# worldfnd/provekit

Measured on AMD Instinct MI355X. Metric: proofs/sec (noir-r1cs prove hot path, WHIR commit + sumcheck + folding rounds), higher is better.
Workload: dtype u32x8 (BN254-Fr, 256-bit Montgomery integers); 1 GPU; poseidon-rounds size class: m=21, m_0=20, satisfiable synthetic R1CS (786429 constraints, 1048571 witnesses, a constant term in half of the rows of A and B), batch-2 WHIR commit + zk-sumcheck + 4-round WHIR opening, queries [109, 28, 16, 11]/9, pow_bits [19.0, 16.0, 16.0, 18.0]/11.0 (WhirConfig::new derivation, security 128, ConjectureList), blinding WHIR n=8 queries [122]/31, Skyscraper-sponge tr; launcher=single process

## Files before the change

### provekit_amd/csrc/internal.hpp

```cpp
#pragma once
#include "ctx.hpp"
#include "rng_core.hpp"

namespace pk {

int ensure_scratch(pk_ctx* ctx, size_t bytes);
int ensure_pinned(pk_ctx* ctx);
int ensure_ws(pk_ctx* ctx, size_t bytes);
enum { PK_HOOK_GATE_SPINS = 0, PK_HOOK_GATE_STALL_US = 1, PK_HOOK_RCCL_SAME_DEVICE = 2, PK_HOOK_COUNT = 3 };
long test_hook(int which);
hipError_t wait_stream(int device, hipStream_t stream);
hipError_t wait_ctx(pk_ctx* ctx);
int wait_ctx_rc(pk_ctx* ctx);
int sync_stream(pk_ctx* ctx);
int mail_alloc(pk_ctx* ctx, size_t bytes, void** out);

int comm_rank(const pk_ctx* ctx);
int comm_world(const pk_ctx* ctx);
int comm_all_gather(pk_ctx* ctx, const void* d_send, void* d_recv, size_t bytes_per_rank);
int comm_all_reduce_sum_u64(pk_ctx* ctx, uint64_t* d_buf, size_t count);
int comm_collect_fe(pk_ctx* ctx, int K, uint64_t* host_out);
int red_across_begin(pk_ctx* ctx);
bool comm_collective_pending(const pk_ctx* ctx);
bool comm_rccl(const pk_ctx* ctx);
hipError_t comm_wait(pk_ctx* ctx);
void comm_turn_begin(pk_ctx* ctx);
void comm_turn_end(pk_ctx* ctx);
unsigned long long comm_collectives_issued(const pk_ctx* ctx);
void comm_abort(pk_ctx* ctx);
void comm_release(pk_ctx* ctx);

int leaf_hash_x(pk_ctx* ctx, const uint64_t* d_leaves, size_t n_leaves, size_t width, uint64_t* d_digests, bool scaled_in);
int merkle_top_x(pk_ctx* ctx, uint64_t* d_nodes, size_t top_leaves);
int read_root(pk_ctx* ctx, const uint64_t* d_nodes, size_t n_leaves, uint64_t root[4]);

void ntt_retain_ctx(pk_ctx* ctx);
void ntt_release_ctx(pk_ctx* ctx);
bool ntt_scaled_available(unsigned log_n);
int rs_encode_x(pk_ctx* ctx, const uint64_t* const* d_coeffs, unsigned batch, unsigned n_vars, unsigned log_inv_rate, unsigned fold,
                uint64_t* d_leaves, uint64_t* d_scratch, bool scaled);
int rs_encode_shard_x(pk_ctx* ctx, const uint64_t* const* d_coeffs, unsigned batch, unsigned n_vars, unsigned log_inv_rate, unsigned fold,
                      unsigned shard, unsigned n_shards, uint64_t* d_leaves_local, uint64_t* d_scratch, bool scaled);

int pow_solve_x(pk_ctx* ctx, const uint8_t challenge[32], double bits, uint64_t* nonce, bool striped);

unsigned shard_factor(const pk_ctx* ctx, size_t rows);
size_t commit_scratch_fes(const pk_ctx* ctx, size_t rows, size_t width);
int commit_into(pk_ctx* ctx, const uint64_t* const* d_coeffs, unsigned batch, unsigned n_vars, unsigned log_inv_rate, unsigned fold,
                uint64_t* d_leaves, uint64_t* d_nodes, uint64_t* d_scratch, pk_commit_layout* layout_out);
int open_raw(pk_ctx* ctx, const uint64_t* d_leaves, const uint64_t* d_nodes, size_t n_leaves, size_t width, const pk_commit_layout& lay,
             const uint64_t* indices, size_t k, int canonical_leaves, uint64_t* leaves_out, uint64_t* sibling_digests, uint64_t* auth_paths);

int eval_univariate_multi(pk_ctx* ctx, const uint64_t* const* d_polys, unsigned np, size_t n, const uint64_t z[4], uint64_t* out);
int dot_rows(pk_ctx* ctx, const uint64_t* d_w, size_t row_stride, unsigned nrows, const uint64_t* d_f, const uint64_t* d_g, size_t n, uint64_t* out,
             bool defer = false);
int lincomb2(pk_ctx* ctx, uint64_t* d_out, const uint64_t* d_a, const uint64_t* beta, const uint64_t* d_b, size_t n);
int lincomb2_pair(pk_ctx* ctx, uint64_t* d_out0, const uint64_t* d_a0, const uint64_t* d_b0, size_t n0, uint64_t* d_out1, const uint64_t* d_a1,
                  const uint64_t* d_b1, size_t n1, const uint64_t* beta);
int axpy3(pk_ctx* ctx, uint64_t* d_y, const uint64_t* g3, const uint64_t* d_rows, size_t row_stride, size_t n);
int to_coeffs_generated(pk_ctx* ctx, unsigned m, const uint64_t* d_wit, size_t n_wit, const RngKey& key, uint32_t stream_mask, uint32_t stream_g,
                        uint64_t* d_f_evals, uint64_t* d_g_evals, uint64_t* d_f_coeffs, uint64_t* d_g_coeffs);
int fold_pairs2(pk_ctx* ctx, const uint64_t* d_v0, uint64_t* d_out0, const uint64_t* d_v1, uint64_t* d_out1, size_t len, const uint64_t* r,
                unsigned gate_seq = 0);
enum class CubicWeight { EqArray, Level };
int sumcheck_cubic_launch(pk_ctx* ctx, uint64_t* d_a, uint64_t* d_b, uint64_t* d_c, CubicWeight kind, uint64_t* d_weight, size_t len,
                          const uint64_t* fold_or_null, unsigned gate_seq, unsigned* red_seq_out);
int sumcheck_quadratic_launch(pk_ctx* ctx, const uint64_t* d_f, const uint64_t* d_w, size_t len, const uint64_t* fold_or_null, unsigned gate_seq,
                              uint64_t* d_f_out, uint64_t* d_w_out, int nsums, unsigned* red_seq_out);
void sumcheck_quadratic_from_claim(const uint64_t claim[4], uint64_t out[12]);
int eq_suffix_tables(pk_ctx* ctx, const uint64_t* r, unsigned n, uint64_t* d_out);
void sumcheck_spliteq_correct(const uint64_t P[4], const uint64_t r_i[4], uint64_t out[12]);
void sumcheck_spliteq_advance(uint64_t P[4], const uint64_t r_i[4], const uint64_t alpha_i[4]);
int sumcheck_collect_spin(pk_ctx* ctx, int nsums, unsigned red_seq, uint64_t out[12]);
int sumcheck_collect(pk_ctx* ctx, int nsums, uint64_t out[12]);
unsigned sumcheck_gate_next(pk_ctx* ctx);
void sumcheck_gate_publish(pk_ctx* ctx, unsigned gate_seq, const uint64_t challenge[4]);
int sumcheck_gate_check(pk_ctx* ctx);
void sumcheck_gate_clear(pk_ctx* ctx);

int witness_bounds_strided(pk_ctx* ctx, const pk_r1cs* r, const uint64_t* d_z, unsigned m0, unsigned stride, unsigned offset, uint64_t* d_a,
                           uint64_t* d_b, uint64_t* d_c);
int external_row_range(pk_ctx* ctx, const pk_r1cs* r, const uint64_t* d_eq_alpha, size_t first, size_t last, uint64_t* d_out);

enum { RNG_MASK = 1, RNG_G = 2, RNG_BLIND = 3, RNG_MASK_B = 4, RNG_G_B = 5, RNG_FILL = 6 };
int proof_key(pk_ctx* ctx, const uint8_t* rng_seed32, RngKey& key);
int random_fe(pk_ctx* ctx, uint64_t* d_out, size_t n, const RngKey& key, uint32_t stream);

void witness_program_shape(const pk_witness_program* p, size_t* n_witnesses, size_t* n_challenges, size_t* n_acir);
// ... 13 lines not shown
```

### provekit_amd/csrc/mle.hip

```cpp
#define PK_BASE_PRIO 2
#include "internal.hpp"
#include "fe29.hpp"
#include "reduce.hpp"

using namespace pk;

namespace {

struct fe_arg {
    u32 v[8];
};
__device__ __forceinline__ fe from_arg(const fe_arg& a) {
    fe r;
#pragma unroll
    for (int i = 0; i < 8; i++) r.v[i] = a.v[i];
    return r;
}
inline fe_arg to_arg(const uint64_t* h) {
    fe_arg a;
    memcpy(a.v, h, 32);
    return a;
}

__device__ __forceinline__ fe lds_get(const uint4* lo, const uint4* hi, int i) {
// ... 310 lines not shown
    PK_LATENCY_PRIO();
    static_assert(NS == 2 || NS == 3, "two or three sums");
    const fe r = (FOLD && gate.host) ? gate_wait(gate) : from_arg(fold_arg);
    fe acc[NS];
#pragma unroll
    for (int q = 0; q < NS; q++) acc[q] = fe_zero();
    const size_t npairs = out_len / 2;
    const size_t stride = (size_t)gridDim.x * blockDim.x;
    for (size_t i = (size_t)blockIdx.x * blockDim.x + threadIdx.x; i < npairs; i += stride) {
        fe f0, f1, w0, w1;
        if (FOLD) {
            fe x0 = fe_load(f + 4 * i), x1 = fe_load(f + 4 * i + 1), x2 = fe_load(f + 4 * i + 2), x3 = fe_load(f + 4 * i + 3);
            f0 = fe_fold(x0, x1, r);
            f1 = fe_fold(x2, x3, r);
            fe y0 = fe_load(w + 4 * i), y1 = fe_load(w + 4 * i + 1), y2 = fe_load(w + 4 * i + 2), y3 = fe_load(w + 4 * i + 3);
            w0 = fe_fold(y0, y1, r);
            w1 = fe_fold(y2, y3, r);
            fe_store(f_out + 2 * i, f0);
            fe_store(f_out + 2 * i + 1, f1);
            fe_store(w_out + 2 * i, w0);
            fe_store(w_out + 2 * i + 1, w1);
        } else {
            f0 = fe_load(f + 2 * i);
            f1 = fe_load(f + 2 * i + 1);
            w0 = fe_load(w + 2 * i);
            w1 = fe_load(w + 2 * i + 1);
        }
        acc[0] = fe_add(acc[0], fe_mulx(f0, w0));
        if (NS == 3) acc[1] = fe_add(acc[1], fe_mulx(f1, w1));
        acc[NS - 1] = fe_add(acc[NS - 1], fe_mulx(fe_sub(fe_dbl(f1), f0), fe_sub(fe_dbl(w1), w0)));
    }
    grid_finish_fe<NS>(acc, red);
}
constexpr size_t SMALL_ROUND_PAIRS = 16384;
constexpr unsigned EQ_SUFFIX_ONE_WG_VARS = 11;

template <CubicWeight W>
__device__ __forceinline__ void cubic_round_small(fe* __restrict__ a, fe* __restrict__ b, fe* __restrict__ c, weight_elem<W>* __restrict__ wt, size_t len,
                                                  fe_arg fold_arg, gate_args gate, red_out red) {
    constexpr bool LEVEL = W == CubicWeight::Level;
    PK_LATENCY_PRIO();
    __shared__ uint4 xs[2 * RED_THREADS];
    const fe alpha = gate.host ? gate_wait(gate) : from_arg(fold_arg);
    const size_t npairs = len / 4, off = npairs, foff = len / 2;
    const unsigned tid = threadIdx.x, g = tid >> 3, role = tid & 7, k = role >> 1, which = role & 1;
    const size_t i = (size_t)blockIdx.x * (RED_THREADS / 8) + g;
    fe* arr = k == 0 ? a : k == 1 ? b : c;
    if constexpr (!LEVEL) arr = k == 0 ? a : k == 1 ? b : k == 2 ? c : wt;
    if (i < npairs && (!LEVEL || k < 3)) {
        fe* p = arr + i + (which ? off : 0);
        fe x = fe_load(p), x2 = fe_load(p + foff);
        x = fe_fold(x, x2, alpha);
        fe_store(p, x);
        lds_put(xs, xs + RED_THREADS, tid, x);
    } else if (LEVEL && i < npairs && role == 6) {
        lds_put(xs, xs + RED_THREADS, tid, fe_load(wt + i));
    }
    __syncthreads();
    fe acc[3] = {fe_zero(), fe_zero(), fe_zero()};
    if (i < npairs && role < 3) {
        const unsigned base = tid & ~7u;
        auto v = [&](unsigned kk, unsigned w) { return lds_get(xs, xs + RED_THREADS, base + 2 * kk + w); };
        const fe a0 = v(0, 0), a1 = v(0, 1), b0 = v(1, 0), b1 = v(1, 1), c0 = v(2, 0), c1 = v(2, 1), e0 = v(3, 0);
        fe e1;
        if constexpr (!LEVEL) e1 = v(3, 1);
        auto pick = [&](const fe& x0, const fe& x1) {
// ... 116 lines not shown
                                                                                   red_out red) {
    cubic_round_small<CubicWeight::Level>(a, b, c, E, len, fold_arg, gate, red);
}

__global__ void fold_pairs_kernel(const fe* __restrict__ v0, fe* __restrict__ out0, const fe* __restrict__ v1, fe* __restrict__ out1,
                                  size_t out_len, fe_arg r_arg, gate_args gate) {
    PK_LATENCY_PRIO();
    const fe r = gate.host ? gate_wait(gate) : from_arg(r_arg);
    const fe* v = blockIdx.y ? v1 : v0;
    fe* out = blockIdx.y ? out1 : out0;
    const size_t stride = (size_t)gridDim.x * blockDim.x;
    for (size_t i = (size_t)blockIdx.x * blockDim.x + threadIdx.x; i < out_len; i += stride) {
        fe x0 = fe_load(v + 2 * i), x1 = fe_load(v + 2 * i + 1);
        fe_store(out + i, fe_fold(x0, x1, r));
    }
}

template <int NV>
__global__ __launch_bounds__(RED_THREADS) void dot_kernel(const fe* __restrict__ w, const fe* __restrict__ f, const fe* __restrict__ g,
                                                          size_t n, red_out red) {
    PK_LATENCY_PRIO();
    fe acc[NV];
#pragma unroll
    for (int k = 0; k < NV; k++) acc[k] = fe_zero();
    const size_t stride = (size_t)gridDim.x * blockDim.x;
    for (size_t i = (size_t)blockIdx.x * blockDim.x + threadIdx.x; i < n; i += stride) {
        fe wi = fe_load(w + i);
        acc[0] = fe_add(acc[0], fe_mulx(wi, fe_load(f + i)));
        if (NV == 2) acc[NV - 1] = fe_add(acc[NV - 1], fe_mulx(wi, fe_load(g + i)));
    }
    grid_finish_fe<NV>(acc, red);
}

template <int NR, int NV>
__global__ __launch_bounds__(RED_THREADS) void dot_rows_kernel(const fe* __restrict__ w, size_t row_stride, const fe* __restrict__ f,
                                                               const fe* __restrict__ g, size_t n, red_out red) {
    PK_LATENCY_PRIO();
    fe acc[NR * NV];
#pragma unroll
    for (int k = 0; k < NR * NV; k++) acc[k] = fe_zero();
    const size_t stride = (size_t)gridDim.x * blockDim.x;
    for (size_t i = (size_t)blockIdx.x * blockDim.x + threadIdx.x; i < n; i += stride) {
        const fe fi = fe_load(f + i);
        fe gi = fi;
        if (NV == 2) gi = fe_load(g + i);
#pragma unroll
        for (int k = 0; k < NR; k++) {
            const fe wi = fe_load(w + (size_t)k * row_stride + i);
            acc[NV * k] = fe_add(acc[NV * k], fe_mulx(wi, fi));
            if (NV == 2) acc[NV * k + 1] = fe_add(acc[NV * k + 1], fe_mulx(wi, gi));
        }
    }
    grid_finish_fe<NR * NV>(acc, red);
}

struct pow2_args {
    fe_arg p[28];
};
__global__ __launch_bounds__(RED_THREADS) void zpow_table_kernel(pow2_args zp, fe* __restrict__ ztab) {
    PK_LATENCY_PRIO();
    fe h = fe_one();
#pragma unroll 1
    for (int i = 0; i < 8; i++)
        if ((threadIdx.x >> i) & 1u) h = fe_mulx(h, from_arg(zp.p[i]));
    fe_store(ztab + threadIdx.x, h);
}
template <int NP>
__global__ __launch_bounds__(RED_THREADS) void horner_kernel(const fe* __restrict__ c, const fe* __restrict__ c_second, size_t n, size_t cnt, pow2_args zp,
                                                             const fe* __restrict__ ztab, red_out red) {
    PK_LATENCY_PRIO();
    __shared__ unsigned s_zb[8];
    static_assert(RED_THREADS == 256, "the lane table has 256 entries");
    const size_t base = (size_t)blockIdx.x * cnt * RED_THREADS;
    if (threadIdx.x == 0) {
        fe zb = fe_one();
        bool any = false;
// ... 88 lines not shown
        if (j == 0 && t < n_out) fe_store(out + t, wide_reduce(w));
    }
}

__global__ __launch_bounds__(256) void lincomb_kernel(fe* __restrict__ out, const fe* __restrict__ a, const fe* __restrict__ b, size_t n,
                                                      fe_arg beta_arg) {
    PK_LATENCY_PRIO();
    const fe beta = from_arg(beta_arg);
    const size_t stride = (size_t)gridDim.x * blockDim.x;
    for (size_t i = (size_t)blockIdx.x * blockDim.x + threadIdx.x; i < n; i += stride)
        fe_store(out + i, fe_add(fe_load(a + i), fe_mulx(beta, fe_load(b + i))));
}
__global__ __launch_bounds__(256) void axpy_kernel(fe* __restrict__ y, const fe* __restrict__ x, size_t n, fe_arg beta_arg) {
    PK_LATENCY_PRIO();
    const fe beta = from_arg(beta_arg);
    const size_t stride = (size_t)gridDim.x * blockDim.x;
    for (size_t i = (size_t)blockIdx.x * blockDim.x + threadIdx.x; i < n; i += stride)
        fe_store(y + i, fe_add(fe_load(y + i), fe_mulx(beta, fe_load(x + i))));
}

__global__ __launch_bounds__(256) void lincomb_pair_kernel(fe* __restrict__ out0, const fe* __restrict__ a0, const fe* __restrict__ b0, size_t n0,
                                                           fe* __restrict__ out1, const fe* __restrict__ a1, const fe* __restrict__ b1, size_t n1,
                                                           fe_arg beta_arg) {
    PK_LATENCY_PRIO();
    const fe beta = from_arg(beta_arg);
    fe* out = blockIdx.y ? out1 : out0;
    const fe* a = blockIdx.y ? a1 : a0;
    const fe* b = blockIdx.y ? b1 : b0;
    const size_t n = blockIdx.y ? n1 : n0;
    const size_t stride = (size_t)gridDim.x * blockDim.x;
    for (size_t i = (size_t)blockIdx.x * blockDim.x + threadIdx.x; i < n; i += stride)
        fe_store(out + i, fe_add(fe_load(a + i), fe_mulx(beta, fe_load(b + i))));
}
struct fe3_arg {
    fe_arg g[3];
};
__global__ __launch_bounds__(256) void axpy3_kernel(fe* __restrict__ y, const fe* __restrict__ rows, size_t row_stride, size_t n, fe3_arg ga) {
    PK_LATENCY_PRIO();
    const fe29 g0 = unpack29<5>(from_arg(ga.g[0])), g1 = unpack29<5>(from_arg(ga.g[1])), g2 = unpack29<5>(from_arg(ga.g[2]));
    const size_t stride = (size_t)gridDim.x * blockDim.x;
    for (size_t i = (size_t)blockIdx.x * blockDim.x + threadIdx.x; i < n; i += stride) {
        dot29 d;
        dot29_init(d);
        dot29_add(d, unpack29<0>(fe_load(rows + i)), g0);
        dot29_add(d, unpack29<0>(fe_load(rows + row_stride + i)), g1);
        dot29_add(d, unpack29<0>(fe_load(rows + 2 * row_stride + i)), g2);
        fe_store(y + i, fe_add(fe_load(y + i), dot29_result(d)));
    }
}

int dot(pk_ctx* ctx, int nv, const uint64_t* d_w, const uint64_t* d_f, const uint64_t* d_g, size_t n, uint64_t* out) {
    if (n == 0) return reduce_empty(ctx, nv, out);
    red_out red;
    unsigned blocks;
    int rc = reduction_begin(ctx, n, &red, &blocks);
    if (rc) return rc;
    {
        ProfScope prof(ctx, "dot");
        auto kernel = nv == 2 ? dot_kernel<2> : dot_kernel<1>;
        kernel<<<blocks, RED_THREADS, 0, ctx->stream>>>((const fe*)d_w, (const fe*)d_f, (const fe*)d_g, n, red);
    }
    PK_LAUNCH_CHECK(ctx);
    return collect_reduction(ctx, nv, out);
}

struct round_launch {
    red_out red;
    unsigned blocks;
    gate_args gate;
// ... 197 lines not shown
    if (!ctx->d_ztab) PK_HIP(ctx, hipMalloc(&ctx->d_ztab, 256 * 32));
    pow2_args zp;
    {
        fe b;
        memcpy(b.v, z, 32);
        for (int i = 0; i < 28; i++) {
            memcpy(zp.p[i].v, b.v, 32);
            b = fe_mulx(b, b);
        }
    }
    {
        ProfScope prof(ctx, "eval_univariate");
        zpow_table_kernel<<<1, RED_THREADS, 0, ctx->stream>>>(zp, (fe*)ctx->d_ztab);
        auto kernel = np == 2 ? horner_kernel<2> : horner_kernel<1>;
        kernel<<<blocks, RED_THREADS, 0, ctx->stream>>>((const fe*)d_polys[0], (const fe*)(np == 2 ? d_polys[1] : nullptr), n, cnt, zp,
                                                        (const fe*)ctx->d_ztab, red);
    }
    PK_LAUNCH_CHECK(ctx);
    return collect_reduction(ctx, (int)np, out);
}
int dot_rows(pk_ctx* ctx, const uint64_t* d_w, size_t row_stride, unsigned nrows, const uint64_t* d_f, const uint64_t* d_g, size_t n, uint64_t* out,
             bool defer) {
    const int nv = d_g ? 2 : 1;
    PK_REQUIRE(ctx, nrows == 3 && (out || defer) && (n == 0 || (d_w && d_f)), "three weight rows");
    PK_REQUIRE(ctx, !defer || (n != 0 && !ctx->red_across), "a deferred dot product needs work and a lone context");
    if (n == 0) return reduce_empty(ctx, 3 * nv, out);
    red_out red;
    unsigned blocks;
    int rc = reduction_begin(ctx, n, &red, &blocks);
    if (rc) return rc;
    {
        ProfScope prof(ctx, "dot");
        auto kernel = nv == 2 ? dot_rows_kernel<3, 2> : dot_rows_kernel<3, 1>;
        kernel<<<blocks, RED_THREADS, 0, ctx->stream>>>((const fe*)d_w, row_stride, (const fe*)d_f, (const fe*)d_g, n, red);
    }
    PK_LAUNCH_CHECK(ctx);
    if (defer) return PK_OK;
    return collect_reduction(ctx, 3 * nv, out);
}

}

extern "C" {

int pk_to_coeffs(pk_ctx* ctx, uint64_t* d_evals, unsigned n_vars) {
    PK_ENTER(ctx);
    return wavelet<true>(ctx, nullptr, d_evals, n_vars);
}
int pk_to_evals(pk_ctx* ctx, uint64_t* d_coeffs, unsigned n_vars) {
    PK_ENTER(ctx);
    return wavelet<false>(ctx, nullptr, d_coeffs, n_vars);
}
int pk_to_coeffs_into(pk_ctx* ctx, const uint64_t* d_src, uint64_t* d_dst, unsigned n_vars) {
    PK_ENTER(ctx);
    PK_REQUIRE(ctx, d_src && d_src != d_dst, "source must differ from destination");
    return wavelet<true>(ctx, d_src, d_dst, n_vars);
}
int pk_to_evals_into(pk_ctx* ctx, const uint64_t* d_src, uint64_t* d_dst, unsigned n_vars) {
    PK_ENTER(ctx);
    PK_REQUIRE(ctx, d_src && d_src != d_dst, "source must differ from destination");
    return wavelet<false>(ctx, d_src, d_dst, n_vars);
}

int pk_eq_accumulate(pk_ctx* ctx, uint64_t* d_w, unsigned n_vars, const uint64_t* points, const uint64_t* scales, unsigned q,
                     int overwrite) {
    PK_ENTER(ctx);
    PK_REQUIRE(ctx, d_w && (q == 0 || (points && scales)), "null pointer");
    PK_REQUIRE(ctx, n_vars <= 30, "too many variables");
    const size_t n = (size_t)1 << n_vars;
    if (q == 0) {
        if (overwrite) PK_HIP(ctx, hipMemsetAsync(d_w, 0, 32 * n, ctx->stream));
        return PK_OK;
    }
    const unsigned nlo = (n_vars + 1) / 2, nhi = n_vars - nlo;
    const size_t per_pt = ((size_t)1 << nhi) + ((size_t)1 << nlo);
    int rc = ensure_ws(ctx, 32 * (size_t)q * per_pt + 64);
    if (rc) return rc;
    PK_REQUIRE(ctx, nlo <= 16, "too many variables");
    char* mail = nullptr;
    rc = mail_alloc(ctx, 32 * ((size_t)q * n_vars + q), (void**)&mail);
    if (rc) return rc;
    fe* d_points = (fe*)mail;
    fe* d_scales = d_points + (size_t)q * n_vars;
    fe* d_tables = (fe*)ctx->d_ws;
    if (n_vars) memcpy(d_points, points, 32 * (size_t)q * n_vars);
    memcpy(d_scales, scales, 32 * (size_t)q);
    {
        ProfScope prof(ctx, "eq_accumulate");
        eq_half_tables_kernel<<<dim3(q, 2), 256, 0, ctx->stream>>>(d_points, d_scales, n_vars, nhi, nlo, d_tables);
        eq_accumulate_kernel<<<grid_for(ctx, nlo ? (n + 1) / 2 : n, 256), 256, 0, ctx->stream>>>((fe*)d_w, n, nhi, nlo, q, d_tables, overwrite);
    }
    PK_LAUNCH_CHECK(ctx);
    return PK_OK;
}

int pk_eq_table(pk_ctx* ctx, const uint64_t* r, unsigned m, uint64_t* d_out) {
    PK_ENTER(ctx);
    static const uint64_t one[4] = {0xac96341c4ffffffbULL, 0x36fc76959f60cd29ULL, 0x666ea36f7879462eULL, 0x0e0a77c19a07df2fULL};
    return pk_eq_accumulate(ctx, d_out, m, r, one, 1, 1);
}


int pk_sumcheck_cubic_round(pk_ctx* ctx, uint64_t* d_a, uint64_t* d_b, uint64_t* d_c, uint64_t* d_eq, size_t len,
                            const uint64_t* fold_or_null, uint64_t out[12]) {
    PK_ENTER(ctx);
    PK_REQUIRE(ctx, out, "null pointer");
    unsigned seq = 0;
    int rc = sumcheck_cubic_launch(ctx, d_a, d_b, d_c, CubicWeight::EqArray, d_eq, len, fold_or_null, 0, &seq);
    if (rc) return rc;
    return collect_reduction(ctx, 3, out);
}

int pk_sumcheck_quadratic_round(pk_ctx* ctx, const uint64_t* d_f, const uint64_t* d_w, size_t len, const uint64_t* fold_or_null,
                                uint64_t* d_f_out, uint64_t* d_w_out, uint64_t out[12]) {
    PK_ENTER(ctx);
    PK_REQUIRE(ctx, out, "null pointer");
    unsigned seq = 0;
    int rc = sumcheck_quadratic_launch(ctx, d_f, d_w, len, fold_or_null, 0, d_f_out, d_w_out, 3, &seq);
    if (rc) return rc;
    return collect_reduction(ctx, 3, out);
}

// ... 105 lines not shown
```

### provekit_amd/csrc/prover.hip

```cpp
#include <unistd.h>

#include <algorithm>
#include <chrono>
#include <cstdlib>
#include <string>
#include <vector>

#include "internal.hpp"
#include "shard_map.hpp"
#include "prover_transcript.hpp"

using namespace pk;

struct pk_scheme {
    const pk_r1cs* r1cs = nullptr;
    size_t num_constraints = 0, num_witnesses = 0;
    unsigned m = 0, m_0 = 0;
    unsigned nb = 0;
    pk_whir_config whir_witness{}, whir_hiding{};
    char* arena = nullptr;
    size_t arena_bytes = 0;
    std::string domain_separator;
    char* noir_witness = nullptr;
    pk_ctx* side = nullptr;
// ... 280 lines not shown
    const unsigned n, k, G, lgG, rank;
    bool sharded;
    const size_t B0, off0;
    fe* d_c = nullptr;
    fe* bp[2] = {};
    fe* bw[2] = {};
    fe* gathered[4] = {};
    int cur = 0;
    size_t len;
    std::vector<fe> rs;
    fe claim;
    bool have_claim = false;
    std::vector<fe> all_r;

    WhirProver(pk_ctx* c, Arena& a, const pk_whir_config& cf, const Commitment& com, Transcript& t)
        : ctx(c), A(a), cfg(cf), C(com), T(t), n(cf.n_vars), k(cf.folding_factor), G((unsigned)comm_world(c)), lgG(ilog2(G)),
          rank((unsigned)comm_rank(c)), sharded(whir_sharded(c, n)), B0(sharded ? ((size_t)1 << n) / G : (size_t)1 << n),
          off0(sharded ? (size_t)rank * B0 : 0), len(B0) {}

    int batch_combine(fe* dst, fe* const* x, size_t from, size_t cnt) {
        if (C.batch == 1) return pk_memcpy_d2d(ctx, dst, x[0] + from, 32 * cnt);
        uint64_t s[4];
        h_store(s, C.beta);
        int rc = lincomb2(ctx, U(dst), U(x[0] + from), s, U(x[1] + from), cnt);
        fe bp_ = h_mul(C.beta, C.beta);
        for (unsigned b = 2; b < C.batch && !rc; b++) {
            h_store(s, bp_);
            rc = pk_fe_axpy(ctx, U(dst), s, U(x[b] + from), cnt);
            bp_ = h_mul(bp_, C.beta);
        }
        return rc;
    }

    int eq_weights(fe* dst, unsigned nv, const std::vector<fe>& zs, const fe& gamma, int overwrite, fe* next) {
        const size_t q = zs.size();
        const unsigned lg = sharded ? lgG : 0, nl = nv - lg;
        std::vector<fe> x(nv ? nv : 1), pts(q * (nl ? nl : 1)), scales(q ? q : 1);
        fe g = fe_one();
        for (size_t j = 0; j < q; j++) {
            expand_from_univariate(zs[j], nv, x.data());
            scales[j] = lg ? h_mul(g, eq_bits(x.data(), lg, rank)) : g;
            std::copy(x.begin() + lg, x.begin() + nv, pts.begin() + j * nl);
            g = h_mul(g, gamma);
        }
        *next = g;
        return pk_eq_accumulate(ctx, U(dst), nl, (const uint64_t*)pts.data(), (const uint64_t*)scales.data(), (unsigned)q, overwrite);
    }

    void flip() {
        cur = 1 - cur;
        len /= 2;
    }

    int sumcheck_rounds(unsigned rounds) {
        rs.clear();
        ns0 = have_claim ? 2 : 3;
        const bool pipelined = ctx->latency_mode && G == 1 && rounds && len >= ((size_t)1 << rounds);
        return sumcheck_round_loop(ctx, T, rounds, pipelined, *this);
    }
    int ns0 = 3;
    int nsums(unsigned t) const { return t ? 2 : ns0; }
    int launch(unsigned t, const uint64_t* fold, unsigned gate_seq, unsigned* red_seq) {
        CK(sumcheck_quadratic_launch(ctx, U(bp[cur]), U(bw[cur]), len, fold, gate_seq, U(bp[1 - cur]), U(bw[1 - cur]), nsums(t), red_seq));
        if (fold || gate_seq) flip();
        return PK_OK;
    }
    bool closing_fold() const { return len >= 2; }
    int fold(const uint64_t* r, unsigned gate_seq) {
        CK(fold_pairs2(ctx, U(bp[cur]), U(bp[1 - cur]), U(bw[cur]), U(bw[1 - cur]), len, r, gate_seq));
        flip();
        return PK_OK;
    }
    int before_sync_launch() { return PK_OK; }
    void meanwhile(unsigned) {}
    unsigned message(unsigned t, uint64_t out[12], fe msg[4]) {
        if (nsums(t) == 2) {
            uint64_t cl[4];
            h_store(cl, claim);
            sumcheck_quadratic_from_claim(cl, out);
        }
        for (int q = 0; q < 3; q++) msg[q] = h_load(out + 4 * q);
        return 3;
    }
    void record(unsigned, const fe* msg, const fe& r) {
        rs.push_back(r);
        all_r.push_back(r);
        claim = eval_quadratic_012(msg, r);
        have_claim = true;
    }

    int gather(fe* p0, fe* p1, fe* w0, fe* w1) {
        CK(gather_blocks(ctx, bp[cur], len, p0));
        CK(gather_blocks(ctx, bw[cur], len, w0));
        bp[0] = p0; bp[1] = p1; bw[0] = w0; bw[1] = w1;
        cur = 0;
        len *= G;
        sharded = false;
        return PK_OK;
    }
    int maybe_gather() { return sharded && len <= SHARD_MIN_LOCAL ? gather(gathered[0], gathered[1], gathered[2], gathered[3]) : PK_OK; }

    int start(fe* const* d_weights, const size_t* weight_len, unsigned n_weights, const fe* weight_sums) {
        const size_t N = (size_t)1 << n;
        ALLOC(dc, N);
        d_c = dc;
        ALLOC(p0, B0);
        ALLOC(p1, B0 / 2 ? B0 / 2 : 1);
        ALLOC(w0, B0);
        ALLOC(w1, B0 / 2 ? B0 / 2 : 1);
        bp[0] = p0; bp[1] = p1; bw[0] = w0; bw[1] = w1;
        bool have_evals = true;
        for (unsigned b = 0; b < C.batch; b++) have_evals = have_evals && C.evals[b] != nullptr;
        const bool pair = have_evals && C.batch == 2;
        if (pair) {
            uint64_t s[4];
            h_store(s, C.beta);
            CK(lincomb2_pair(ctx, U(d_c), U(C.polys[0]), U(C.polys[1]), N, U(p0), U(C.evals[0] + off0), U(C.evals[1] + off0), B0, s));
        } else {
            CK(batch_combine(d_c, C.polys, 0, N));
        }
        if (have_evals) {
            if (!pair) CK(batch_combine(p0, C.evals, off0, B0));
        } else if (!sharded) {
            CK(pk_to_evals_into(ctx, U(d_c), U(p0), n));
        } else {
            ALLOC(d_ev, N);
            CK(pk_to_evals_into(ctx, U(d_c), U(d_ev), n));
            CK(pk_memcpy_d2d(ctx, p0, d_ev + off0, 32 * B0));
        }
        const fe gamma = T.challenge_scalar();
        fe g;
        CK(eq_weights(w0, n, C.ood_points, gamma, 1, &g));
        auto batched = [&](const fe* v, size_t step) {
            fe acc = v[0], bb = C.beta;
            for (unsigned b = 1; b < C.batch; b++, bb = h_mul(bb, C.beta)) acc = h_add(acc, h_mul(bb, v[b * step]));
            return acc;
        };
        const size_t q = C.ood_points.size();
        claim = fe_zero();
        fe gq = fe_one();
        for (size_t j = 0; j < q; j++, gq = h_mul(gq, gamma)) claim = h_add(claim, h_mul(gq, batched(&C.ood_answers[j], q)));
        have_claim = weight_sums || !n_weights;
        const bool rows3 = rows_at_equal_stride3(d_weights, weight_len, n_weights);
        if (rows3) {
            uint64_t s3[12];
            fe g3 = g;
            for (int i = 0; i < 3; i++, g3 = h_mul(g3, gamma)) h_store(s3 + 4 * i, g3);
            CK(axpy3(ctx, U(w0), s3, U(d_weights[0] + off0), (size_t)(d_weights[1] - d_weights[0]), in_block(weight_len[0], off0, B0)));
        }
        for (unsigned i = 0; i < n_weights; i++) {
            uint64_t s[4];
            h_store(s, g);
            const size_t cnt = in_block(weight_len[i], off0, B0);
            if (cnt && !rows3) CK(pk_fe_axpy(ctx, U(w0), s, U(d_weights[i] + off0), cnt));
            if (weight_sums) claim = h_add(claim, h_mul(g, batched(weight_sums + (size_t)i * C.batch, 1)));
            g = h_mul(g, gamma);
        }
        if (sharded) {
            const size_t cap = G * SHARD_MIN_LOCAL;
            const size_t sizes[4] = {cap, cap / 2, cap, cap / 2};
            for (int q = 0; q < 4; q++) {
                ALLOC(buf, sizes[q]);
                gathered[q] = buf;
            }
        }
        CK(sumcheck_rounds(k));
        return maybe_gather();
    }

    int rounds() {
        const Commitment* prev = &C;
        Commitment com;
        unsigned nv = n, log_inv_rate = cfg.starting_log_inv_rate;
        size_t domain_size = (size_t)1 << (n + log_inv_rate);
        fe exp_gen = folded_domain_generator(n + log_inv_rate, k);
        for (unsigned r = 0; r < cfg.n_rounds; r++) {
            const unsigned nv2 = nv - k;
            ALLOC(d_c2, (size_t)1 << nv2);
            CK(pk_fold_coeffs(ctx, U(d_c), nv, (const uint64_t*)rs.data(), k, U(d_c2)));
            d_c = d_c2;
            nv = nv2;
            log_inv_rate += k - 1;
            Commitment next;
            CK(whir_commit_compute(ctx, A, nv, log_inv_rate, k, &d_c, 1, next));
            fe root;
            CK(read_root(ctx, U(next.nodes), next.rows, (uint64_t*)root.v));
            T.add_canon(root);
            std::vector<fe> zs(cfg.ood_samples[r]);
            T.challenge_scalars(zs.data(), zs.size());
            std::vector<fe> ood_ans(zs.size());
            for (size_t j = 0; j < zs.size(); j++) CK(eval_univariate_x(ctx, d_c, (size_t)1 << nv, zs[j], ood_ans[j]));
            T.add_scalars(ood_ans.data(), ood_ans.size());
            CK(pow_round(ctx, T, cfg.pow_bits[r]));
            const std::vector<uint64_t> idx = stir_queries(T, domain_size, k, cfg.num_queries[r]);
            CK(emit_opening_hints(ctx, T, *prev, idx));
            const fe gamma = T.challenge_scalar();
            for (uint64_t i : idx) zs.push_back(h_pow(exp_gen, i));
            fe g;
            CK(eq_weights(bw[cur], nv, zs, gamma, 0, &g));
            have_claim = false;
            CK(sumcheck_rounds(k));
            CK(maybe_gather());
            com = next;
            prev = &com;
            domain_size /= 2;
            exp_gen = h_mul(exp_gen, exp_gen);
        }
        return final_round(*prev, nv, domain_size);
    }

    int final_round(const Commitment& prev, unsigned nv, size_t domain_size) {
        if (sharded) {
            const size_t cap = len * G;
            ALLOC(fp0, cap);
            ALLOC(fp1, cap / 2 ? cap / 2 : 1);
            ALLOC(fw0, cap);
            ALLOC(fw1, cap / 2 ? cap / 2 : 1);
            CK(gather(fp0, fp1, fw0, fw1));
        }
        const unsigned nv2 = nv - k;
        ALLOC(d_final, (size_t)1 << nv2);
        CK(pk_fold_coeffs(ctx, U(d_c), nv, (const uint64_t*)rs.data(), k, U(d_final)));
        std::vector<fe> fin((size_t)1 << nv2);
        CK(pk_memcpy_d2h(ctx, fin.data(), d_final, 32 * fin.size()));
        T.add_scalars(fin.data(), fin.size());
        CK(pow_round(ctx, T, cfg.final_pow_bits));
        const std::vector<uint64_t> idx = stir_queries(T, domain_size, k, cfg.final_queries);
        CK(emit_opening_hints(ctx, T, prev, idx));
        CK(sumcheck_rounds(nv2));
        return pow_round(ctx, T, cfg.final_folding_pow_bits);
    }

    int deferred_hint(fe* const* d_weights, const size_t* weight_len, unsigned n_weights) {
        if (!n_weights) return PK_OK;
        std::vector<fe> point(all_r.rbegin(), all_r.rend());
        const bool sh = whir_sharded(ctx, n);
        ALLOC(d_eq, B0);
        if (sh) {
            const fe sc = eq_bits(point.data(), lgG, rank);
            CK(pk_eq_accumulate(ctx, U(d_eq), n - lgG, (const uint64_t*)(point.data() + lgG), (const uint64_t*)&sc, 1, 1));
        } else {
            CK(pk_eq_table(ctx, (const uint64_t*)point.data(), n, U(d_eq)));
        }
        Across ac(ctx, sh);
        CK(ac.rc);
        std::vector<fe> evals(n_weights);
        const bool rows3 = rows_at_equal_stride3(d_weights, weight_len, n_weights);
        if (rows3) {
            uint64_t o[12] = {};
            if (sh || weight_len[0])
                CK(dot_rows(ctx, U(d_weights[0] + off0), (size_t)(d_weights[1] - d_weights[0]), 3, U(d_eq), nullptr, in_block(weight_len[0], off0, B0), o));
            for (int i = 0; i < 3; i++) evals[i] = h_load(o + 4 * i);
        } else {
            for (unsigned i = 0; i < n_weights; i++) {
                uint64_t o[4] = {};
                if (sh || weight_len[i]) CK(pk_dot(ctx, U(d_weights[i] + off0), U(d_eq), in_block(weight_len[i], off0, B0), o));
                evals[i] = h_load(o);
            }
        }
        std::vector<uint8_t> buf;
        put_vec(buf, evals.data(), n_weights);
        T.hint(buf.data(), buf.size());
        return PK_OK;
    }
};
int whir_prove(pk_ctx* ctx, Arena& A, const pk_whir_config& cfg, const Commitment& C, fe* const* d_weights, const size_t* weight_len,
               unsigned n_weights, const fe* weight_sums, Transcript& T) {
    WhirProver P(ctx, A, cfg, C, T);
    CK(P.start(d_weights, weight_len, n_weights, weight_sums));
    CK(P.rounds());
    return P.deferred_hint(d_weights, weight_len, n_weights);
}

struct BatchCommit {
    Commitment com;
    fe* f_evals = nullptr;
    fe* g_evals = nullptr;
};
int batch_commit_compute(pk_ctx* ctx, Arena& A, unsigned m, const pk_whir_config& cfg, const fe* d_evals, size_t n_evals, const RngKey& key,
                         u32 stream_mask, u32 stream_g, BatchCommit& out) {
    const size_t half = (size_t)1 << (m - 1), N = 2 * half;
    ALLOC(f, N);
    ALLOC(g, N);
    ALLOC(fe_, N);
    ALLOC(ge_, N);
    if (comm_world(ctx) <= 1) {
        CK(to_coeffs_generated(ctx, m, U(d_evals), n_evals, key, stream_mask, stream_g, U(f), U(g), U(fe_), U(ge_)));
    } else {
        CK(pk_memset_zero(ctx, f, 32 * half));
        CK(pk_memcpy_d2d(ctx, f, d_evals, 32 * n_evals));
// ... 489 lines not shown
```

Before: 286.1 proofs/s.

## Fuse WHIR opening weight build, batch combine and first sumcheck round into one kernel

```diff
diff --git a/provekit_amd/csrc/internal.hpp b/provekit_amd/csrc/internal.hpp
--- a/provekit_amd/csrc/internal.hpp
+++ b/provekit_amd/csrc/internal.hpp
@@ -54,6 +54,22 @@
 int eval_univariate_multi(pk_ctx* ctx, const uint64_t* const* d_polys, unsigned np, size_t n, const uint64_t z[4], uint64_t* out);
 int dot_rows(pk_ctx* ctx, const uint64_t* d_w, size_t row_stride, unsigned nrows, const uint64_t* d_f, const uint64_t* d_g, size_t n, uint64_t* out,
              bool defer = false);
+int dot_rows_eq(pk_ctx* ctx, const uint64_t* d_w, size_t row_stride, unsigned nrows, const uint64_t* point, unsigned n_vars, size_t n, uint64_t* out);
+struct opening_first {
+    const uint64_t *d_e0, *d_e1, *beta;
+    uint64_t *d_p, *d_w;
+    size_t n;
+    const uint64_t *points, *scales;
+    unsigned q;
+    int overwrite;
+    const uint64_t* d_rows;
+    size_t row_stride;
+    unsigned nrows;
+    size_t row_len;
+    const uint64_t* row_scales;
+    int nsums;
+};
+int opening_first_launch(pk_ctx* ctx, const opening_first& a, unsigned grid, unsigned* red_seq_out);
 int lincomb2(pk_ctx* ctx, uint64_t* d_out, const uint64_t* d_a, const uint64_t* beta, const uint64_t* d_b, size_t n);
 int lincomb2_pair(pk_ctx* ctx, uint64_t* d_out0, const uint64_t* d_a0, const uint64_t* d_b0, size_t n0, uint64_t* d_out1, const uint64_t* d_a1,
                   const uint64_t* d_b1, size_t n1, const uint64_t* beta);
diff --git a/provekit_amd/csrc/mle.hip b/provekit_amd/csrc/mle.hip
--- a/provekit_amd/csrc/mle.hip
+++ b/provekit_amd/csrc/mle.hip
@@ -366,6 +366,80 @@
     }
     grid_finish_fe<NS>(acc, red);
 }
+struct fe3_arg {
+    fe_arg g[3];
+};
+struct first_rows {
+    const fe* rows;
+    size_t stride, len;
+    fe3_arg g;
+};
+template <int NR>
+__device__ __forceinline__ fe first_rows_term(const first_rows& R, size_t i) {
+    static_assert(NR == 1 || NR == 3, "one row or three");
+    if constexpr (NR == 1) {
+        return fe_mulx(from_arg(R.g.g[0]), fe_load(R.rows + i));
+    } else {
+        dot29 d;
+        dot29_init(d);
+#pragma unroll
+        for (int k = 0; k < 3; k++) dot29_add(d, unpack29<0>(fe_load(R.rows + k * R.stride + i)), unpack29<5>(from_arg(R.g.g[k])));
+        return dot29_result(d);
+    }
+}
+template <bool COMBINE, int NR, int NS>
+__global__ __launch_bounds__(RED_THREADS) void opening_first_kernel(const fe* __restrict__ e0, const fe* __restrict__ e1, fe_arg beta_arg,
+                                                                    fe* __restrict__ p, fe* __restrict__ w, size_t n, unsigned nhi, unsigned nlo,
+                                                                    unsigned q, const fe* __restrict__ tables, int overwrite, first_rows R, red_out red) {
+    PK_LATENCY_PRIO();
+    static_assert(NS == 2 || NS == 3, "two or three sums");
+    const size_t per_pt = ((size_t)1 << nhi) + ((size_t)1 << nlo);
+    const size_t mask = ((size_t)1 << nlo) - 1;
+    fe acc[NS];
+#pragma unroll
+    for (int s = 0; s < NS; s++) acc[s] = fe_zero();
+    const size_t stride = (size_t)gridDim.x * blockDim.x;
+    for (size_t j = (size_t)blockIdx.x * blockDim.x + threadIdx.x; j < n / 2; j += stride) {
+        const size_t i = 2 * j;
+        dot29 d0, d1;
+        dot29_init(d0);
+        dot29_init(d1);
+        const fe* T = tables;
+        for (unsigned pt = 0; pt < q; pt++, T += per_pt) {
+            const fe29 h = unpack29<0>(fe_load(T + (i >> nlo)));
+            const fe* lo = T + ((size_t)1 << nhi) + (i & mask);
+            dot29_add(d0, h, unpack29<5>(fe_load(lo)));
+            dot29_add(d1, h, unpack29<5>(fe_load(lo + 1)));
+        }
+        fe w0 = dot29_result(d0), w1 = dot29_result(d1);
+        if (!overwrite) {
+            w0 = fe_add(fe_load(w + i), w0);
+            w1 = fe_add(fe_load(w + i + 1), w1);
+        }
+        if constexpr (NR > 0) {
+            if (i < R.len) w0 = fe_add(w0, first_rows_term<NR>(R, i));
+            if (i + 1 < R.len) w1 = fe_add(w1, first_rows_term<NR>(R, i + 1));
+        }
+        fe_store(w + i, w0);
+        fe_store(w + i + 1, w1);
+        fe f0, f1;
+        if constexpr (COMBINE) {
+            const fe beta = from_arg(beta_arg);
+            f0 = fe_add(fe_load(e0 + i), fe_mulx(beta, fe_load(e1 + i)));
+            f1 = fe_add(fe_load(e0 + i + 1), fe_mulx(beta, fe_load(e1 + i + 1)));
+            fe_store(p + i, f0);
+            fe_store(p + i + 1, f1);
+        } else {
+            f0 = fe_load(p + i);
+            f1 = fe_load(p + i + 1);
+        }
+        acc[0] = fe_add(acc[0], fe_mulx(f0, w0));
+        if (NS == 3) acc[1] = fe_add(acc[1], fe_mulx(f1, w1));
+        acc[NS - 1] = fe_add(acc[NS - 1], fe_mulx(fe_sub(fe_dbl(f1), f0), fe_sub(fe_dbl(w1), w0)));
+    }
+    grid_finish_fe<NS>(acc, red);
+}
+
 constexpr size_t SMALL_ROUND_PAIRS = 16384;
 constexpr unsigned EQ_SUFFIX_ONE_WG_VARS = 11;
 
@@ -548,16 +622,19 @@
     grid_finish_fe<NV>(acc, red);
 }
 
-template <int NR, int NV>
+template <int NR, int NV, bool EQF = false>
 __global__ __launch_bounds__(RED_THREADS) void dot_rows_kernel(const fe* __restrict__ w, size_t row_stride, const fe* __restrict__ f,
-                                                               const fe* __restrict__ g, size_t n, red_out red) {
-    PK_LATENCY_PRIO();
+                                                               const fe* __restrict__ g, size_t n, unsigned nhi, unsigned nlo, red_out red) {
+    PK_LATENCY_PRIO();
+    static_assert(!EQF || NV == 1, "the equality table stands in for f alone");
     fe acc[NR * NV];
 #pragma unroll
     for (int k = 0; k < NR * NV; k++) acc[k] = fe_zero();
     const size_t stride = (size_t)gridDim.x * blockDim.x;
     for (size_t i = (size_t)blockIdx.x * blockDim.x + threadIdx.x; i < n; i += stride) {
-        const fe fi = fe_load(f + i);
+        fe fi;
+        if constexpr (EQF) fi = fe_mulx(fe_load(f + (i >> nlo)), fe_load(f + ((size_t)1 << nhi) + (i & (((size_t)1 << nlo) - 1))));
+        else fi = fe_load(f + i);
         fe gi = fi;
         if (NV == 2) gi = fe_load(g + i);
 #pragma unroll
@@ -712,9 +789,6 @@
     for (size_t i = (size_t)blockIdx.x * blockDim.x + threadIdx.x; i < n; i += stride)
         fe_store(out + i, fe_add(fe_load(a + i), fe_mulx(beta, fe_load(b + i))));
 }
-struct fe3_arg {
-    fe_arg g[3];
-};
 __global__ __launch_bounds__(256) void axpy3_kernel(fe* __restrict__ y, const fe* __restrict__ rows, size_t row_stride, size_t n, fe3_arg ga) {
     PK_LATENCY_PRIO();
     const fe29 g0 = unpack29<5>(from_arg(ga.g[0])), g1 = unpack29<5>(from_arg(ga.g[1])), g2 = unpack29<5>(from_arg(ga.g[2]));
@@ -978,11 +1052,92 @@
     {
         ProfScope prof(ctx, "dot");
         auto kernel = nv == 2 ? dot_rows_kernel<3, 2> : dot_rows_kernel<3, 1>;
-        kernel<<<blocks, RED_THREADS, 0, ctx->stream>>>((const fe*)d_w, row_stride, (const fe*)d_f, (const fe*)d_g, n, red);
+        kernel<<<blocks, RED_THREADS, 0, ctx->stream>>>((const fe*)d_w, row_stride, (const fe*)d_f, (const fe*)d_g, n, 0, 0, red);
     }
     PK_LAUNCH_CHECK(ctx);
     if (defer) return PK_OK;
     return collect_reduction(ctx, 3 * nv, out);
+}
+
+namespace {
+int eq_half_tables(pk_ctx* ctx, unsigned n_vars, const uint64_t* points, const uint64_t* scales, unsigned q, unsigned* nhi_out, unsigned* nlo_out,
+                   const fe** d_tables) {
+    const unsigned nlo = (n_vars + 1) / 2, nhi = n_vars - nlo;
+    PK_REQUIRE(ctx, n_vars <= 30 && nlo <= 16, "too many variables");
+    *nhi_out = nhi;
+    *nlo_out = nlo;
+    *d_tables = nullptr;
+    if (!q) return PK_OK;
+    const size_t per_pt = ((size_t)1 << nhi) + ((size_t)1 << nlo);
+    int rc = ensure_ws(ctx, 32 * (size_t)q * per_pt + 64);
+    if (rc) return rc;
+    char* mail = nullptr;
+    rc = mail_alloc(ctx, 32 * ((size_t)q * n_vars + q), (void**)&mail);
+    if (rc) return rc;
+    fe* d_points = (fe*)mail;
+    fe* d_scales = d_points + (size_t)q * n_vars;
+    if (n_vars) memcpy(d_points, points, 32 * (size_t)q * n_vars);
+    memcpy(d_scales, scales, 32 * (size_t)q);
+    eq_half_tables_kernel<<<dim3(q, 2), 256, 0, ctx->stream>>>(d_points, d_scales, n_vars, nhi, nlo, (fe*)ctx->d_ws);
+    *d_tables = (const fe*)ctx->d_ws;
+    return PK_OK;
+}
+}
+
+int opening_first_launch(pk_ctx* ctx, const opening_first& a, unsigned grid, unsigned* red_seq_out) {
+    PK_REQUIRE(ctx, a.d_p && a.d_w && red_seq_out && (a.nsums == 2 || a.nsums == 3), "null pointer");
+    PK_REQUIRE(ctx, is_pow2(a.n) && a.n >= 2, "size must be a power of two >= 2");
+    PK_REQUIRE(ctx, a.q == 0 || (a.points && a.scales), "null pointer");
+    const bool combine = a.d_e0 != nullptr;
+    PK_REQUIRE(ctx, !combine || (a.d_e1 && a.beta), "null pointer");
+    PK_REQUIRE(ctx, a.nrows == 0 || ((a.nrows == 1 || a.nrows == 3) && a.row_scales && (a.row_len == 0 || a.d_rows) && a.row_len <= a.n), "one row or three");
+    PK_REQUIRE(ctx, combine == (a.nrows != 0) && (combine || a.nsums == 3), "either the opening's first launch (combination and rows) or a round's (neither, three sums)");
+    unsigned nhi, nlo;
+    const fe* d_tables;
+    ProfScope prof(ctx, "opening_first");
+    int rc = eq_half_tables(ctx, ilog2(a.n), a.points, a.scales, a.q, &nhi, &nlo, &d_tables);
+    if (rc) return rc;
+    const size_t npairs = a.n / 2;
+    red_out red;
+    unsigned blocks;
+    rc = reduction_begin(ctx, npairs, &red, &blocks);
+    if (rc) return rc;
+    *red_seq_out = red.seq;
+    const size_t want = (npairs + RED_THREADS - 1) / RED_THREADS;
+    blocks = (unsigned)(want < (size_t)RED_MAX_BLOCKS ? want : (size_t)RED_MAX_BLOCKS);
+    if (grid && grid < blocks) blocks = grid;
+    first_rows R{(const fe*)a.d_rows, a.row_stride, a.row_len, {}};
+    for (unsigned k = 0; k < a.nrows; k++) R.g.g[k] = to_arg(a.row_scales + 4 * k);
+    using kernel_t = void (*)(const fe*, const fe*, fe_arg, fe*, fe*, size_t, unsigned, unsigned, unsigned, const fe*, int, first_rows, red_out);
+    kernel_t kernel = opening_first_kernel<false, 0, 3>;
+    if (combine && a.nrows == 1) kernel = a.nsums == 2 ? opening_first_kernel<true, 1, 2> : opening_first_kernel<true, 1, 3>;
+    if (combine && a.nrows == 3) kernel = a.nsums == 2 ? opening_first_kernel<true, 3, 2> : opening_first_kernel<true, 3, 3>;
+    kernel<<<blocks, RED_THREADS, 0, ctx->stream>>>((const fe*)a.d_e0, (const fe*)a.d_e1, combine ? to_arg(a.beta) : fe_arg{}, (fe*)a.d_p, (fe*)a.d_w, a.n,
+                                                    nhi, nlo, a.q, d_tables, a.overwrite, R, red);
+    PK_LAUNCH_CHECK(ctx);
+    return PK_OK;
+}
+
+int dot_rows_eq(pk_ctx* ctx, const uint64_t* d_w, size_t row_stride, unsigned nrows, const uint64_t* point, unsigned n_vars, size_t n, uint64_t* out) {
+    PK_REQUIRE(ctx, (nrows == 1 || nrows == 3) && out && point && (n == 0 || d_w), "one weight row or three");
+    PK_REQUIRE(ctx, n <= ((size_t)1 << n_vars), "rows longer than the table");
+    if (n == 0) return reduce_empty(ctx, (int)nrows, out);
+    static const uint64_t one[4] = {0xac96341c4ffffffbULL, 0x36fc76959f60cd29ULL, 0x666ea36f7879462eULL, 0x0e0a77c19a07df2fULL};
+    unsigned nhi, nlo;
+    const fe* d_tables;
+    int rc = eq_half_tables(ctx, n_vars, point, one, 1, &nhi, &nlo, &d_tables);
+    if (rc) return rc;
+    red_out red;
+    unsigned blocks;
+    rc = reduction_begin(ctx, n, &red, &blocks);
+    if (rc) return rc;
+    {
+        ProfScope prof(ctx, "dot");
+        auto kernel = nrows == 3 ? dot_rows_kernel<3, 1, true> : dot_rows_kernel<1, 1, true>;
+        kernel<<<blocks, RED_THREADS, 0, ctx->stream>>>((const fe*)d_w, row_stride, d_tables, nullptr, n, nhi, nlo, red);
+    }
+    PK_LAUNCH_CHECK(ctx);
+    return collect_reduction(ctx, (int)nrows, out);
 }
 
 }
@@ -1018,22 +1173,12 @@
         if (overwrite) PK_HIP(ctx, hipMemsetAsync(d_w, 0, 32 * n, ctx->stream));
         return PK_OK;
     }
-    const unsigned nlo = (n_vars + 1) / 2, nhi = n_vars - nlo;
-    const size_t per_pt = ((size_t)1 << nhi) + ((size_t)1 << nlo);
-    int rc = ensure_ws(ctx, 32 * (size_t)q * per_pt + 64);
-    if (rc) return rc;
-    PK_REQUIRE(ctx, nlo <= 16, "too many variables");
-    char* mail = nullptr;
-    rc = mail_alloc(ctx, 32 * ((size_t)q * n_vars + q), (void**)&mail);
-    if (rc) return rc;
-    fe* d_points = (fe*)mail;
-    fe* d_scales = d_points + (size_t)q * n_vars;
-    fe* d_tables = (fe*)ctx->d_ws;
-    if (n_vars) memcpy(d_points, points, 32 * (size_t)q * n_vars);
-    memcpy(d_scales, scales, 32 * (size_t)q);
+    unsigned nhi, nlo;
+    const fe* d_tables;
     {
         ProfScope prof(ctx, "eq_accumulate");
-        eq_half_tables_kernel<<<dim3(q, 2), 256, 0, ctx->stream>>>(d_points, d_scales, n_vars, nhi, nlo, d_tables);
+        int rc = eq_half_tables(ctx, n_vars, points, scales, q, &nhi, &nlo, &d_tables);
+        if (rc) return rc;
         eq_accumulate_kernel<<<grid_for(ctx, nlo ? (n + 1) / 2 : n, 256), 256, 0, ctx->stream>>>((fe*)d_w, n, nhi, nlo, q, d_tables, overwrite);
     }
     PK_LAUNCH_CHECK(ctx);
diff --git a/provekit_amd/csrc/prover.hip b/provekit_amd/csrc/prover.hip
--- a/provekit_amd/csrc/prover.hip
+++ b/provekit_amd/csrc/prover.hip
@@ -336,10 +336,14 @@
         return rc;
     }
 
-    int eq_weights(fe* dst, unsigned nv, const std::vector<fe>& zs, const fe& gamma, int overwrite, fe* next) {
+    int eq_weights(fe* dst, unsigned nv, const std::vector<fe>& zs, const fe& gamma, int overwrite, fe* next, bool defer = false) {
         const size_t q = zs.size();
         const unsigned lg = sharded ? lgG : 0, nl = nv - lg;
-        std::vector<fe> x(nv ? nv : 1), pts(q * (nl ? nl : 1)), scales(q ? q : 1);
+        std::vector<fe> x(nv ? nv : 1);
+        std::vector<fe>& pts = first.pts;
+        std::vector<fe>& scales = first.scales;
+        pts.assign(q * (nl ? nl : 1), fe_zero());
+        scales.assign(q ? q : 1, fe_zero());
         fe g = fe_one();
         for (size_t j = 0; j < q; j++) {
             expand_from_univariate(zs[j], nv, x.data());
@@ -348,8 +352,23 @@
             g = h_mul(g, gamma);
         }
         *next = g;
-        return pk_eq_accumulate(ctx, U(dst), nl, (const uint64_t*)pts.data(), (const uint64_t*)scales.data(), (unsigned)q, overwrite);
-    }
+        if (!defer) return pk_eq_accumulate(ctx, U(dst), nl, (const uint64_t*)pts.data(), (const uint64_t*)scales.data(), (unsigned)q, overwrite);
+        first.a = opening_first{};
+        first.a.d_w = U(dst);
+        first.a.n = (size_t)1 << nl;
+        first.a.points = (const uint64_t*)pts.data();
+        first.a.scales = (const uint64_t*)scales.data();
+        first.a.q = (unsigned)q;
+        first.a.overwrite = overwrite;
+        first.pending = true;
+        return PK_OK;
+    }
+    struct First {
+        bool pending = false;
+        opening_first a{};
+        std::vector<fe> pts, scales;
+        uint64_t beta[4], row_scales[12];
+    } first;
 
     void flip() {
         cur = 1 - cur;
@@ -365,6 +384,12 @@
     int ns0 = 3;
     int nsums(unsigned t) const { return t ? 2 : ns0; }
     int launch(unsigned t, const uint64_t* fold, unsigned gate_seq, unsigned* red_seq) {
+        if (first.pending) {
+            first.pending = false;
+            first.a.d_p = U(bp[cur]);
+            first.a.nsums = nsums(t);
+            return opening_first_launch(ctx, first.a, 0, red_seq);
+        }
         CK(sumcheck_quadratic_launch(ctx, U(bp[cur]), U(bw[cur]), len, fold, gate_seq, U(bp[1 - cur]), U(bw[1 - cur]), nsums(t), red_seq));
         if (fold || gate_seq) flip();
         return PK_OK;
@@ -416,7 +441,12 @@
         bool have_evals = true;
         for (unsigned b = 0; b < C.batch; b++) have_evals = have_evals && C.evals[b] != nullptr;
         const bool pair = have_evals && C.batch == 2;
-        if (pair) {
+        const bool rows3 = rows_at_equal_stride3(d_weights, weight_len, n_weights);
+        const bool fused = pair && !sharded && B0 >= 2 && k >= 1 && (rows3 || n_weights == 1) && weight_len[0] <= B0;
+        if (fused) {
+            h_store(first.beta, C.beta);
+            CK(lincomb2(ctx, U(d_c), U(C.polys[0]), first.beta, U(C.polys[1]), N));
+        } else if (pair) {
             uint64_t s[4];
             h_store(s, C.beta);
             CK(lincomb2_pair(ctx, U(d_c), U(C.polys[0]), U(C.polys[1]), N, U(p0), U(C.evals[0] + off0), U(C.evals[1] + off0), B0, s));
@@ -434,7 +464,7 @@
         }
         const fe gamma = T.challenge_scalar();
         fe g;
-        CK(eq_weights(w0, n, C.ood_points, gamma, 1, &g));
+        CK(eq_weights(w0, n, C.ood_points, gamma, 1, &g, fused));
         auto batched = [&](const fe* v, size_t step) {
             fe acc = v[0], bb = C.beta;
             for (unsigned b = 1; b < C.batch; b++, bb = h_mul(bb, C.beta)) acc = h_add(acc, h_mul(bb, v[b * step]));
@@ -445,8 +475,18 @@
         fe gq = fe_one();
         for (size_t j = 0; j < q; j++, gq = h_mul(gq, gamma)) claim = h_add(claim, h_mul(gq, batched(&C.ood_answers[j], q)));
         have_claim = weight_sums || !n_weights;
-        const bool rows3 = rows_at_equal_stride3(d_weights, weight_len, n_weights);
-        if (rows3) {
+        if (fused) {
+            fe g3 = g;
+            for (unsigned i = 0; i < n_weights; i++, g3 = h_mul(g3, gamma)) h_store(first.row_scales + 4 * i, g3);
+            first.a.d_e0 = U(C.evals[0]);
+            first.a.d_e1 = U(C.evals[1]);
+            first.a.beta = first.beta;
+            first.a.d_rows = U(d_weights[0]);
+            first.a.row_stride = rows3 ? (size_t)(d_weights[1] - d_weights[0]) : 0;
+            first.a.nrows = n_weights;
+            first.a.row_len = weight_len[0];
+            first.a.row_scales = first.row_scales;
+        } else if (rows3) {
             uint64_t s3[12];
             fe g3 = g;
             for (int i = 0; i < 3; i++, g3 = h_mul(g3, gamma)) h_store(s3 + 4 * i, g3);
@@ -456,7 +496,7 @@
             uint64_t s[4];
             h_store(s, g);
             const size_t cnt = in_block(weight_len[i], off0, B0);
-            if (cnt && !rows3) CK(pk_fe_axpy(ctx, U(w0), s, U(d_weights[i] + off0), cnt));
+            if (cnt && !rows3 && !fused) CK(pk_fe_axpy(ctx, U(w0), s, U(d_weights[i] + off0), cnt));
             if (weight_sums) claim = h_add(claim, h_mul(g, batched(weight_sums + (size_t)i * C.batch, 1)));
             g = h_mul(g, gamma);
         }
@@ -501,7 +541,7 @@
             const fe gamma = T.challenge_scalar();
             for (uint64_t i : idx) zs.push_back(h_pow(exp_gen, i));
             fe g;
-            CK(eq_weights(bw[cur], nv, zs, gamma, 0, &g));
+            CK(eq_weights(bw[cur], nv, zs, gamma, 0, &g, !sharded && len >= 2 && k >= 1));
             have_claim = false;
             CK(sumcheck_rounds(k));
             CK(maybe_gather());
@@ -539,27 +579,33 @@
         if (!n_weights) return PK_OK;
         std::vector<fe> point(all_r.rbegin(), all_r.rend());
         const bool sh = whir_sharded(ctx, n);
-        ALLOC(d_eq, B0);
-        if (sh) {
-            const fe sc = eq_bits(point.data(), lgG, rank);
-            CK(pk_eq_accumulate(ctx, U(d_eq), n - lgG, (const uint64_t*)(point.data() + lgG), (const uint64_t*)&sc, 1, 1));
-        } else {
-            CK(pk_eq_table(ctx, (const uint64_t*)point.data(), n, U(d_eq)));
-        }
-        Across ac(ctx, sh);
-        CK(ac.rc);
         std::vector<fe> evals(n_weights);
         const bool rows3 = rows_at_equal_stride3(d_weights, weight_len, n_weights);
-        if (rows3) {
+        if (!sh && (rows3 || n_weights == 1)) {
             uint64_t o[12] = {};
-            if (sh || weight_len[0])
+            CK(dot_rows_eq(ctx, U(d_weights[0]), rows3 ? (size_t)(d_weights[1] - d_weights[0]) : 0, n_weights, (const uint64_t*)point.data(), n,
+                           weight_len[0], o));
+            for (unsigned i = 0; i < n_weights; i++) evals[i] = h_load(o + 4 * i);
+        } else {
+            ALLOC(d_eq, B0);
+            if (sh) {
+                const fe sc = eq_bits(point.data(), lgG, rank);
+                CK(pk_eq_accumulate(ctx, U(d_eq), n - lgG, (const uint64_t*)(point.data() + lgG), (const uint64_t*)&sc, 1, 1));
+            } else {
+                CK(pk_eq_table(ctx, (const uint64_t*)point.data(), n, U(d_eq)));
+            }
+            Across ac(ctx, sh);
+            CK(ac.rc);
+            if (rows3) {
+                uint64_t o[12] = {};
                 CK(dot_rows(ctx, U(d_weights[0] + off0), (size_t)(d_weights[1] - d_weights[0]), 3, U(d_eq), nullptr, in_block(weight_len[0], off0, B0), o));
-            for (int i = 0; i < 3; i++) evals[i] = h_load(o + 4 * i);
-        } else {
-            for (unsigned i = 0; i < n_weights; i++) {
-                uint64_t o[4] = {};
-                if (sh || weight_len[i]) CK(pk_dot(ctx, U(d_weights[i] + off0), U(d_eq), in_block(weight_len[i], off0, B0), o));
-                evals[i] = h_load(o);
+                for (int i = 0; i < 3; i++) evals[i] = h_load(o + 4 * i);
+            } else {
+                for (unsigned i = 0; i < n_weights; i++) {
+                    uint64_t o[4] = {};
+                    if (sh || weight_len[i]) CK(pk_dot(ctx, U(d_weights[i] + off0), U(d_eq), in_block(weight_len[i], off0, B0), o));
+                    evals[i] = h_load(o);
+                }
             }
         }
         std::vector<uint8_t> buf;
```

Measured after the change: 289.4 proofs/s, median of 6. 1.01x the previous value.
